# yyNoBug/VAE_segmentation

Hardware: AMD Instinct MI355X
Metric: 3D train-step volumes/sec at 96^3 batch=2 (joint VAE+seg) (higher is better)
Workload: dtype bf16; 1 GPU; configs[1]: 96^3 joint VAE+seg training step (joint_train), batch=2/GPU, bf16 activations + fp32 accumulate, SGD momentum 0.9, VAE frozen, HIP-graph replay; global_batch=2, parallelism=dp1, activation_recomputation=False, tail_in_graph=True, nranks=1, grad_exchange=none (1 rank)

## Files before the change

### vae_segmentation_amd/csrc/pack.hip

```cpp
#include "common.h"

template <typename T>
__device__ __forceinline__ void pack_one(const float* __restrict__ src, T* __restrict__ dst, int d0, int d1, int ntaps,
                                         int c_pad, int form, long long total, long long frag) {
    constexpr int EPL = ET<T>::EPL, KG = ET<T>::KG;
    const long long i = frag * EPL;
    if (i >= total) return;
    float v[EPL];
#pragma unroll
    for (int j = 0; j < EPL; ++j) v[j] = 0.f;
    if (sizeof(T) == 2 && form != VS_PACK_SCATTER_D1 && vs_k3_toeplitz(form == VS_PACK_ROWS_D0 ? d0 : d1, c_pad, ntaps, VS_BF16)) {
        const int lane = (int)(frag & 63), kg = (int)(frag >> 6);
        const int row = lane & 15, dx2 = row >> 3, co = row & 7, tx = (lane >> 4) - dx2;
        if (tx >= 0 && tx <= 2) {
            const int tap = kg * 3 + tx;
#pragma unroll
            for (int ci = 0; ci < EPL; ++ci) {
                if (form == VS_PACK_ROWS_D0) { if (co < d0 && ci < d1) v[ci] = src[((size_t)co * d1 + ci) * 27 + tap]; }
                else { if (co < d1 && ci < d0) v[ci] = src[((size_t)ci * d1 + co) * 27 + (26 - tap)]; }
            }
        }
    } else if (sizeof(T) == 4 && form != VS_PACK_SCATTER_D1 && vs_k3_toeplitz_f32(form == VS_PACK_ROWS_D0 ? d0 : d1, c_pad, ntaps, VS_F32)) {
        const int lane = (int)(frag & 63), kg = (int)(frag >> 6);
        const int row = lane & 15, dy2 = row >> 3, co = row & 7, g = lane >> 4;
        const int t = kg * 2 + (g >> 1), ci0 = (g & 1) * 4;
        const int dz = t / 12, wy = (t / 3) % 4, dx = t % 3, dy = wy - dy2;
        if (dy >= 0 && dy <= 2) {
            const int tap = dz * 9 + dy * 3 + dx;
#pragma unroll
            for (int j = 0; j < EPL; ++j) {
                const int ci = ci0 + j;
                if (form == VS_PACK_ROWS_D0) { if (co < d0 && ci < d1) v[j] = src[((size_t)co * d1 + ci) * 27 + tap]; }
                else { if (co < d1 && ci < d0) v[j] = src[((size_t)ci * d1 + co) * 27 + (26 - tap)]; }
            }
        }
    } else {
        const int CK = c_pad < 32 ? c_pad : 32;
        const int nch = c_pad / CK;
        const int gemm_taps = form == VS_PACK_SCATTER_D1 ? 1 : ntaps;
        const int nkg = (gemm_taps * CK + KG - 1) / KG;
        const unsigned int fr = (unsigned int)frag;
        const int lane = (int)(fr & 63u);
        unsigned int r = fr >> 6;
        const int kg = (int)(r % (unsigned int)nkg); r /= (unsigned int)nkg;
        const int rb = (int)(r / (unsigned int)nch);
        const int ch = (int)(r - (unsigned int)rb * (unsigned int)nch);
        const int row = rb * 16 + (lane & 15);
        const int kk0 = kg * KG + (lane >> 4) * EPL;
        const int tap = kk0 / CK;
        const int c0 = ch * CK + kk0 % CK;
#pragma unroll
        for (int j = 0; j < EPL; ++j) {
            const int c = c0 + j;
            if (form == VS_PACK_ROWS_D0) {
                if (row < d0 && tap < ntaps && c < d1) v[j] = src[((size_t)row * d1 + c) * ntaps + tap];
            } else if (form == VS_PACK_ROWS_D1_FLIP) {
                if (row < d1 && tap < ntaps && c < d0) v[j] = src[((size_t)c * d1 + row) * ntaps + (ntaps - 1 - tap)];
            } else {
                const int t = row / d1, m = row - t * d1;
                if (t < ntaps && tap < 1 && c < d0) v[j] = src[((size_t)c * d1 + m) * ntaps + t];
            }
        }
    }
    *(u32x4*)(dst + i) = frag_pack(v, (T*)nullptr);
}

__device__ __forceinline__ unsigned short limb_of(float v, int limb) {
    const unsigned short b0 = f2bf(v);
    const float r1 = v - bf2f(b0);
    const unsigned short b1 = f2bf(r1);
    return limb == 0 ? b0 : (limb == 1 ? b1 : f2bf(r1 - bf2f(b1)));
}

__device__ __forceinline__ void pack_one_limbs(const float* __restrict__ src, unsigned short* __restrict__ dst, int d0, int d1, int ntaps,
                                               int c_pad, int form, long long total, long long frag, int CK) {
    const long long i = frag * 8;
    if (i >= total) return;
    if (CK < 0) {
        const int lane = (int)(frag & 63), limb = (int)((frag >> 6) % 3), kg = (int)(frag / 192);
        const int row = lane & 15, dx2 = row >> 3, co = row & 7, tx = (lane >> 4) - dx2;
        unsigned short o[8];
#pragma unroll
        for (int ci = 0; ci < 8; ++ci) {
            float v = 0.f;
            if (tx >= 0 && tx <= 2) {
                const int tap = kg * 3 + tx;
                if (form == VS_PACK_ROWS_D0) { if (co < d0 && ci < d1) v = src[((size_t)co * d1 + ci) * 27 + tap]; }
                else { if (co < d1 && ci < d0) v = src[((size_t)ci * d1 + co) * 27 + (26 - tap)]; }
            }
            o[ci] = limb_of(v, limb);
        }
        u32x4 pk;
#pragma unroll
        for (int q = 0; q < 4; ++q) pk[q] = (unsigned int)o[2 * q] | ((unsigned int)o[2 * q + 1] << 16);
        *(u32x4*)(dst + i) = pk;
        return;
    }
    const int nch = c_pad / CK;
    const int nkg = (ntaps * CK + 31) / 32;
    const unsigned int fr = (unsigned int)frag;
    const int lane = (int)(fr & 63u);
    unsigned int r = fr >> 6;
    const int limb = (int)(r % 3u); r /= 3u;
    const int kg = (int)(r % (unsigned int)nkg); r /= (unsigned int)nkg;
    const int rb = (int)(r / (unsigned int)nch);
    const int ch = (int)(r - (unsigned int)rb * (unsigned int)nch);
    const int row = rb * 16 + (lane & 15);
    const int kk0 = kg * 32 + (lane >> 4) * 8;
    const int tap = kk0 / CK;
    const int c0 = ch * CK + kk0 % CK;
    unsigned short o[8];
#pragma unroll
    for (int j = 0; j < 8; ++j) {
        const int c = c0 + j;
        float v = 0.f;
        if (form == VS_PACK_ROWS_D0) { if (row < d0 && tap < ntaps && c < d1) v = src[((size_t)row * d1 + c) * ntaps + tap]; }
        else { if (row < d1 && tap < ntaps && c < d0) v = src[((size_t)c * d1 + row) * ntaps + (ntaps - 1 - tap)]; }
        o[j] = limb_of(v, limb);
    }
    u32x4 pk;
#pragma unroll
    for (int q = 0; q < 4; ++q) pk[q] = (unsigned int)o[2 * q] | ((unsigned int)o[2 * q + 1] << 16);
    *(u32x4*)(dst + i) = pk;
}
__global__ void pack_weight_limbs_kernel(const float* __restrict__ src, unsigned short* __restrict__ dst, int d0, int d1, int ntaps, int c_pad, int form,
                                         long long total, int ck) {
    pack_one_limbs(src, dst, d0, d1, ntaps, c_pad, form, total, (long long)blockIdx.x * blockDim.x + threadIdx.x, ck);
}

template <typename T>
__global__ void pack_weight_kernel(const float* __restrict__ src, T* __restrict__ dst, int d0, int d1, int ntaps,
                                   int c_pad, int form, long long total) {
    pack_one<T>(src, dst, d0, d1, ntaps, c_pad, form, total, (long long)blockIdx.x * blockDim.x + threadIdx.x);
}

__global__ __launch_bounds__(256) void pack_weight_multi_kernel(const vs_pack_desc* __restrict__ descs, int n_desc, int total_blocks, int k3x_ck) {
    const int chunk = (int)gridDim.x >> 3;
    const int lb = ((int)blockIdx.x & 7) * chunk + ((int)blockIdx.x >> 3);
    if (lb >= total_blocks) return;
    __shared__ int s_fb[1024];
    const bool in_lds = n_desc <= 1024;
    if (in_lds) {
        for (int i = threadIdx.x; i < n_desc; i += 256) s_fb[i] = descs[i].first_block;
        __syncthreads();
    }
    int lo = 0, hi = n_desc - 1;
    while (lo < hi) {
        const int mid = (lo + hi + 1) >> 1;
        if ((in_lds ? s_fb[mid] : descs[mid].first_block) <= lb) lo = mid; else hi = mid - 1;
    }
    const vs_pack_desc d = descs[lo];
    const long long i = (long long)(lb - d.first_block) * 256 + threadIdx.x;
    if (d.dtype == VS_F32X3) {
        const int rows = d.form == VS_PACK_ROWS_D0 ? d.d0 : d.d1;
        const bool toep = k3x_ck < 0 ? false : (d.total == 9ll * 3 * 64 * 8 && d.c_pad == 8 && rows <= 8);
        pack_one_limbs(d.src, (unsigned short*)d.dst, d.d0, d.d1, d.ntaps, d.c_pad, d.form, d.total, i, toep ? -1 : (d.c_pad < k3x_ck ? d.c_pad : k3x_ck));
    }
    else if (d.dtype == VS_F32) pack_one<float>(d.src, (float*)d.dst, d.d0, d.d1, d.ntaps, d.c_pad, d.form, d.total, i);
    else if (d.dtype == VS_BF16) pack_one<unsigned short>(d.src, (unsigned short*)d.dst, d.d0, d.d1, d.ntaps, d.c_pad, d.form, d.total, i);
    else pack_one<vs_half>(d.src, (vs_half*)d.dst, d.d0, d.d1, d.ntaps, d.c_pad, d.form, d.total, i);
}

extern "C" int vs_pack_weight_multi(const vs_pack_desc* descs, int n_desc, int total_blocks, void* stream) {
    if (!descs || n_desc <= 0 || total_blocks <= 0) return VS_EINVAL;
    hipLaunchKernelGGL(pack_weight_multi_kernel, dim3(8 * ((total_blocks + 7) / 8)), dim3(256), 0, (hipStream_t)stream, descs, n_desc, total_blocks, vs_k3x_ck(16));
    VS_CHECK_LAUNCH();
    return VS_OK;
}

static long long packed_elems(int rows, int c_pad, int gemm_taps, int dtype) {
    if (dtype == VS_F32X3) {
        if (vs_k3x_toeplitz(rows, c_pad, gemm_taps)) return 9ll * 3 * 64 * 8;
        const int CK = vs_k3x_ck(c_pad);
        return (long long)((rows + 15) / 16) * (c_pad / CK) * ((gemm_taps * CK + 31) / 32) * 3 * 64 * 8;
    }
    if (vs_k3_toeplitz(rows, c_pad, gemm_taps, dtype)) return 9 * 64 * 8;
    if (vs_k3_toeplitz_f32(rows, c_pad, gemm_taps, dtype)) return 18 * 64 * 4;
    const int EPL = dtype == VS_F32 ? 4 : 8, KG = 4 * EPL;
    const int CK = c_pad < 32 ? c_pad : 32;
    const int nch = c_pad / CK;
    const int nkg = (gemm_taps * CK + KG - 1) / KG;
    const int rbt = (rows + 15) / 16;
    return (long long)rbt * nch * nkg * 64 * EPL;
}

extern "C" size_t vs_packed_weight_bytes(int rows, int c_pad, int ntaps, int dtype) {
    return (size_t)packed_elems(rows, c_pad, ntaps, dtype) * (dtype == VS_F32 ? 4 : 2);
}

extern "C" int vs_pack_weight(const float* src, void* dst, int d0, int d1, int ntaps, int c_pad, int form, int dtype,
                              void* stream) {
    if (!src || !dst || d0 <= 0 || d1 <= 0) return VS_EINVAL;
    if (!(c_pad == 8 || c_pad == 16 || (c_pad % 32 == 0 && c_pad > 0))) return VS_ESHAPE;
    if (!vs_dtype_ok(dtype) && dtype != VS_F32X3) return VS_EDTYPE;
    if (dtype == VS_F32X3 && (form == VS_PACK_SCATTER_D1 || ntaps != 27)) return VS_ESHAPE;
    int rows, kc, gemm_taps;
    if (form == VS_PACK_ROWS_D0) { rows = d0; kc = d1; gemm_taps = ntaps; }
    else if (form == VS_PACK_ROWS_D1_FLIP) { rows = d1; kc = d0; gemm_taps = ntaps; }
    else if (form == VS_PACK_SCATTER_D1) { rows = ntaps * d1; kc = d0; gemm_taps = 1; }
    else return VS_EINVAL;
    if (kc > c_pad) return VS_ESHAPE;
    if (!(ntaps == 27 || ntaps == 8)) return VS_ESHAPE;
    const long long total = packed_elems(rows, c_pad, gemm_taps, dtype);
    const int blocks = vs_ceil_div(total / (dtype == VS_F32 ? 4 : 8), 256);
    if (dtype == VS_F32X3) {
        hipLaunchKernelGGL(pack_weight_limbs_kernel, dim3(blocks), dim3(256), 0, (hipStream_t)stream, src, (unsigned short*)dst, d0, d1, ntaps, c_pad, form, total,
                           vs_k3x_toeplitz(rows, c_pad, gemm_taps) ? -1 : vs_k3x_ck(c_pad));
        VS_CHECK_LAUNCH();
        return VS_OK;
    }
    dispatch_t(dtype, [&](auto* tag) {
        using T = TAG_T(tag);
        hipLaunchKernelGGL(pack_weight_kernel<T>, dim3(blocks), dim3(256), 0, (hipStream_t)stream, src, (T*)dst, d0, d1, ntaps, c_pad, form, total);
    });
    VS_CHECK_LAUNCH();
    return VS_OK;
}

template <typename T>
__global__ void pack_planar_kernel(const float* __restrict__ src, T* __restrict__ dst, long long voxels, int c_src,
                                   int c_pad, long long total_vox) {
    const long long i = (long long)blockIdx.x * blockDim.x + threadIdx.x;
    if (i >= total_vox) return;
    const long long n = i / voxels, v = i - n * voxels;
    T* o = dst + i * c_pad;
    for (int c0 = 0; c0 < c_pad; c0 += ET<T>::EPL) {
        float f[ET<T>::EPL];
#pragma unroll
        for (int j = 0; j < ET<T>::EPL; ++j) {
            const int c = c0 + j;
            f[j] = c < c_src ? src[(n * c_src + c) * voxels + v] : 0.f;
        }
        *(u32x4*)(o + c0) = frag_pack(f, (T*)nullptr);
    }
}

template <typename T>
__global__ void unpack_planar_kernel(const T* __restrict__ src, float* __restrict__ dst, long long voxels, int c_dst,
                                     int c_pad, long long total_vox) {
    const long long i = (long long)blockIdx.x * blockDim.x + threadIdx.x;
    if (i >= total_vox) return;
    const long long n = i / voxels, v = i - n * voxels;
    for (int c0 = 0; c0 < c_dst; c0 += ET<T>::EPL) {
        float f[ET<T>::EPL];
        frag_unpack(*(const u32x4*)(src + i * c_pad + c0), f, (T*)nullptr);
#pragma unroll
        for (int j = 0; j < ET<T>::EPL; ++j)
            if (c0 + j < c_dst) dst[(n * c_dst + c0 + j) * voxels + v] = f[j];
    }
}

extern "C" int vs_pack_planar(const float* src, void* dst, int n, long long voxels, int c_src, int c_pad, int dtype,
                              void* stream) {
    if (!src || !dst || n <= 0 || voxels <= 0 || c_src <= 0 || c_src > c_pad || c_pad % 8) return VS_EINVAL;
    const long long tv = (long long)n * voxels;
    if (!vs_dtype_ok(dtype)) return VS_EDTYPE;
    dispatch_t(dtype, [&](auto* tag) {
        using T = TAG_T(tag);
        hipLaunchKernelGGL(pack_planar_kernel<T>, dim3(vs_ceil_div(tv, 256)), dim3(256), 0, (hipStream_t)stream, src, (T*)dst, voxels, c_src, c_pad, tv);
    });
    VS_CHECK_LAUNCH();
    return VS_OK;
}

extern "C" int vs_unpack_planar(const void* src, float* dst, int n, long long voxels, int c_dst, int c_pad, int dtype,
                                void* stream) {
    if (!src || !dst || n <= 0 || voxels <= 0 || c_dst <= 0 || c_dst > c_pad || c_pad % 8) return VS_EINVAL;
    const long long tv = (long long)n * voxels;
    if (!vs_dtype_ok(dtype)) return VS_EDTYPE;
    dispatch_t(dtype, [&](auto* tag) {
        using T = TAG_T(tag);
        hipLaunchKernelGGL(unpack_planar_kernel<T>, dim3(vs_ceil_div(tv, 256)), dim3(256), 0, (hipStream_t)stream, (const T*)src, dst, voxels, c_dst, c_pad, tv);
    });
    VS_CHECK_LAUNCH();
    return VS_OK;
}
```

Baseline: 890.1 volumes/s.

## Stage weight packing through LDS for coalesced source reads in multi-pack kernel

Rewrites the multi-descriptor weight pack kernel so each block first gathers source weights with thread-to-element mapping chosen for contiguous reads, stores them into a padded shared-memory tile, then reads fragments back and writes packed bf16/fp16/fp32/limb outputs. The old path had each thread gather its fragment elements with strided, uncoalesced global loads. This adds a shared-memory buffer, a barrier, and more complex index math, with risk of mismatched layouts for edge cases like toeplitz or scatter forms.

```diff
diff --git a/vae_segmentation_amd/csrc/pack.hip b/vae_segmentation_amd/csrc/pack.hip
--- a/vae_segmentation_amd/csrc/pack.hip
+++ b/vae_segmentation_amd/csrc/pack.hip
@@ -134,11 +134,102 @@
     pack_one<T>(src, dst, d0, d1, ntaps, c_pad, form, total, (long long)blockIdx.x * blockDim.x + threadIdx.x);
 }
 
+enum { PK_GEN = 0, PK_TOEP16 = 1, PK_TOEP32 = 2 };
+
+struct PackGroup { int kg, rb, ch; };
+__device__ __forceinline__ PackGroup pack_group(const vs_pack_desc& d, int kind, int KG, int CK, unsigned int wg) {
+    if (kind != PK_GEN) return PackGroup{(int)wg, 0, 0};
+    const unsigned int nch = (unsigned int)(d.c_pad / CK);
+    const int gemm_taps = (d.form == VS_PACK_SCATTER_D1 && d.dtype != VS_F32X3) ? 1 : d.ntaps;
+    const unsigned int nkg = (unsigned int)((gemm_taps * CK + KG - 1) / KG);
+    const unsigned int r = wg / nkg, rb = r / nch;
+    return PackGroup{(int)(wg - r * nkg), (int)rb, (int)(r - rb * nch)};
+}
+
+__device__ __forceinline__ int pack_src(const vs_pack_desc& d, int kind, int KG, int lCK, const PackGroup& g, int rl, int kl) {
+    const bool rows_d0 = d.form == VS_PACK_ROWS_D0;
+    if (kind != PK_GEN) {
+        const int sh = rl >> 3, co = rl & 7;
+        int tap, ci;
+        if (kind == PK_TOEP16) {
+            const int tx = (kl >> 3) - sh;
+            if (tx < 0 || tx > 2) return -1;
+            tap = g.kg * 3 + tx; ci = kl & 7;
+        } else {
+            const int lg = kl >> 2, t = g.kg * 2 + (lg >> 1);
+            const int dy = (t / 3) % 4 - sh;
+            if (dy < 0 || dy > 2) return -1;
+            tap = (t / 12) * 9 + dy * 3 + t % 3; ci = (lg & 1) * 4 + (kl & 3);
+        }
+        if (rows_d0) return (co < d.d0 && ci < d.d1) ? (co * d.d1 + ci) * 27 + tap : -1;
+        return (co < d.d1 && ci < d.d0) ? (ci * d.d1 + co) * 27 + (26 - tap) : -1;
+    }
+    const int row = g.rb * 16 + rl, kk = g.kg * KG + kl;
+    const int tap = kk >> lCK, c = (g.ch << lCK) + (kk & ((1 << lCK) - 1));
+    if (rows_d0) return (row < d.d0 && tap < d.ntaps && c < d.d1) ? (row * d.d1 + c) * d.ntaps + tap : -1;
+    if (d.form == VS_PACK_SCATTER_D1 && d.dtype != VS_F32X3) {
+        const int t = row / d.d1, m = row - t * d.d1;
+        return (t < d.ntaps && tap < 1 && c < d.d0) ? (c * d.d1 + m) * d.ntaps + t : -1;
+    }
+    return (row < d.d1 && tap < d.ntaps && c < d.d0) ? (c * d.d1 + row) * d.ntaps + (d.ntaps - 1 - tap) : -1;
+}
+
+#define PK_WAVE_PAD 4
+
+template <int EPL>
+__device__ __forceinline__ void pack_block(const vs_pack_desc& d, int blk, int kind, int CK, bool limbs, float* __restrict__ s_v) {
+    constexpr int KG = 4 * EPL, WSTRIDE = 64 * EPL + PK_WAVE_PAD;
+    const int tid = (int)threadIdx.x;
+    const unsigned int g0 = (unsigned int)blk * 4u;
+    const unsigned int ngroups = (unsigned int)(d.total / (64 * EPL));
+    const int TPW = (kind == PK_GEN && KG > CK) ? KG / CK : 1;
+    const int ltp = 31 - __clz(TPW), lck = 31 - __clz(KG / TPW), lCK = 31 - __clz(CK);
+    const int tw = tid & (TPW - 1), w = (tid >> ltp) & 3, r0 = tid >> (ltp + 2);
+    const unsigned int gl = g0 + (unsigned int)w;
+    const bool live = gl < ngroups;
+    const PackGroup pg = pack_group(d, kind, KG, CK, limbs ? gl / 3u : gl);
+    float val[EPL];
+    int at[EPL];
+#pragma unroll
+    for (int it = 0; it < EPL; ++it) {
+        const int rest = it * (64 >> ltp) + r0;
+        const int cl = rest & ((KG >> ltp) - 1), rl = rest >> lck;
+        const int kl = (tw << lck) + cl;
+        const int idx = live ? pack_src(d, kind, KG, lCK, pg, rl, kl) : -1;
+        val[it] = idx >= 0 ? d.src[idx] : 0.f;
+        at[it] = w * WSTRIDE + ((kl / EPL) * 16 + rl) * EPL + kl % EPL;
+    }
+#pragma unroll
+    for (int it = 0; it < EPL; ++it) s_v[at[it]] = val[it];
+    __syncthreads();
+    const unsigned int g = g0 + (unsigned int)(tid >> 6);
+    if (g >= ngroups) return;
+    const float* sv = s_v + (tid >> 6) * WSTRIDE + (tid & 63) * EPL;
+    float v[EPL];
+#pragma unroll
+    for (int q = 0; q < EPL / 4; ++q) {
+        const f32x4 t = *(const f32x4*)(sv + 4 * q);
+        v[4 * q] = t[0]; v[4 * q + 1] = t[1]; v[4 * q + 2] = t[2]; v[4 * q + 3] = t[3];
+    }
+    const size_t i = ((size_t)blk * 256 + tid) * EPL;
+    if constexpr (EPL == 4) *(u32x4*)((float*)d.dst + i) = frag_pack(v, (float*)nullptr);
+    else if (limbs) {
+        const int limb = (int)(g % 3u);
+        u32x4 pk;
+#pragma unroll
+        for (int q = 0; q < 4; ++q) pk[q] = (unsigned int)limb_of(v[2 * q], limb) | ((unsigned int)limb_of(v[2 * q + 1], limb) << 16);
+        *(u32x4*)((unsigned short*)d.dst + i) = pk;
+    }
+    else if (d.dtype == VS_BF16) *(u32x4*)((unsigned short*)d.dst + i) = frag_pack(v, (unsigned short*)nullptr);
+    else *(u32x4*)((vs_half*)d.dst + i) = frag_pack(v, (vs_half*)nullptr);
+}
+
 __global__ __launch_bounds__(256) void pack_weight_multi_kernel(const vs_pack_desc* __restrict__ descs, int n_desc, int total_blocks, int k3x_ck) {
     const int chunk = (int)gridDim.x >> 3;
     const int lb = ((int)blockIdx.x & 7) * chunk + ((int)blockIdx.x >> 3);
     if (lb >= total_blocks) return;
     __shared__ int s_fb[1024];
+    __shared__ __attribute__((aligned(16))) float s_v[4 * (64 * 8 + PK_WAVE_PAD)];
     const bool in_lds = n_desc <= 1024;
     if (in_lds) {
         for (int i = threadIdx.x; i < n_desc; i += 256) s_fb[i] = descs[i].first_block;
@@ -150,15 +241,18 @@
         if ((in_lds ? s_fb[mid] : descs[mid].first_block) <= lb) lo = mid; else hi = mid - 1;
     }
     const vs_pack_desc d = descs[lo];
-    const long long i = (long long)(lb - d.first_block) * 256 + threadIdx.x;
+    const int blk = lb - d.first_block;
+    const int rows = d.form == VS_PACK_ROWS_D0 ? d.d0 : d.d1;
     if (d.dtype == VS_F32X3) {
-        const int rows = d.form == VS_PACK_ROWS_D0 ? d.d0 : d.d1;
         const bool toep = k3x_ck < 0 ? false : (d.total == 9ll * 3 * 64 * 8 && d.c_pad == 8 && rows <= 8);
-        pack_one_limbs(d.src, (unsigned short*)d.dst, d.d0, d.d1, d.ntaps, d.c_pad, d.form, d.total, i, toep ? -1 : (d.c_pad < k3x_ck ? d.c_pad : k3x_ck));
-    }
-    else if (d.dtype == VS_F32) pack_one<float>(d.src, (float*)d.dst, d.d0, d.d1, d.ntaps, d.c_pad, d.form, d.total, i);
-    else if (d.dtype == VS_BF16) pack_one<unsigned short>(d.src, (unsigned short*)d.dst, d.d0, d.d1, d.ntaps, d.c_pad, d.form, d.total, i);
-    else pack_one<vs_half>(d.src, (vs_half*)d.dst, d.d0, d.d1, d.ntaps, d.c_pad, d.form, d.total, i);
+        pack_block<8>(d, blk, toep ? PK_TOEP16 : PK_GEN, d.c_pad < k3x_ck ? d.c_pad : k3x_ck, true, s_v);
+    } else if (d.dtype == VS_F32) {
+        const bool toep = d.form != VS_PACK_SCATTER_D1 && vs_k3_toeplitz_f32(rows, d.c_pad, d.ntaps, VS_F32);
+        pack_block<4>(d, blk, toep ? PK_TOEP32 : PK_GEN, d.c_pad < 32 ? d.c_pad : 32, false, s_v);
+    } else {
+        const bool toep = d.form != VS_PACK_SCATTER_D1 && vs_k3_toeplitz(rows, d.c_pad, d.ntaps, VS_BF16);
+        pack_block<8>(d, blk, toep ? PK_TOEP16 : PK_GEN, d.c_pad < 32 ? d.c_pad : 32, false, s_v);
+    }
 }
 
 extern "C" int vs_pack_weight_multi(const vs_pack_desc* descs, int n_desc, int total_blocks, void* stream) {
```

Measured after the change: 890.1 volumes/s. About the same (-0.0%).
